# Kronuz/Xapiand

Measured on AMD Instinct MI355X. Metric: queries/sec + p50 latency, 10M-doc synthetic index, 3-term AND, top-10, higher is better.
Workload: dtype u32 postings + f64 BM25

## Files before the change

include/xgm.h:

```cpp
#ifndef XGM_H
#define XGM_H

#include <stddef.h>
#include <stdint.h>

#ifdef __cplusplus
extern "C" {
#endif
#if defined(__GNUC__)
#pragma GCC visibility push(default)
#endif

#define XGM_MAX_TERMS 16
#define XGM_MAX_K 1024

#define XGM_OK 0
#define XGM_UNSUPPORTED 1
#define XGM_E_INVALID (-1)
#define XGM_E_IO (-2)
#define XGM_E_NO_DEVICE (-3)
#define XGM_E_DEVICE (-4)
#define XGM_E_REVISION (-5)
#define XGM_E_NOMEM (-6)

// ... 349 lines not shown
int xgm_last_batch_bitmap_skipped(xgm_index*, uint64_t* words);

uint64_t xgm_query_postings_bytes(const xgm_index*, const xgm_query*);

int64_t xgm_debug_decode_term_device(xgm_index*, uint32_t term_id, uint32_t* did, uint32_t* wdf, uint64_t cap);

int64_t xgm_debug_read_doclen(xgm_index*, uint32_t* out, uint64_t cap);

int64_t xgm_debug_read_positions(xgm_index*, uint32_t term_id, uint32_t* out, uint64_t cap);

int64_t xgm_debug_read_container(xgm_index*, uint32_t term_id, uint32_t stripe, unsigned char* out, uint64_t cap, uint32_t* layout);

int xgm_debug_read_wdf_summary(xgm_index*, uint32_t term_id, uint32_t stripe, uint64_t* out);

int xgm_debug_read_term_wdf0(xgm_index*, uint32_t term_id, uint32_t* out);

int64_t xgm_debug_read_flat(xgm_index*, uint32_t term_id, uint32_t* did, unsigned char* wdf, uint32_t* pos, uint64_t cap, uint32_t* has_pos);

double xgm_debug_plan_us(const xgm_index*, const xgm_query_desc* descs, const xgm_global_stats* gs, uint32_t nq, uint32_t reps);

int xgm_debug_batch_launches(const xgm_index*, const xgm_query* qs, uint32_t nq, char* out, uint32_t cap);

int xgm_debug_host_ns(uint64_t* out8);

int xgm_debug_replay_info(uint64_t* out2);
typedef struct {
    uint64_t known_matching_docs;
    double max_weight, frozen_weight;
    uint32_t n_hits, max_weight_subqs, frozen, parallel;
} xgm_replay_figures;
int xgm_debug_replay_list(int device, const xgm_hit* list, uint64_t n, uint32_t k, uint64_t check_at_least, uint32_t mode, uint64_t seg_min,
                          xgm_hit* hits, xgm_replay_figures* out);
int xgm_debug_batch_replay_info(uint64_t* out3);
int xgm_debug_batching_info(const xgm_index*, uint64_t* out3);
double xgm_debug_concurrent_searches(xgm_index*, const xgm_query_desc* descs, const xgm_global_stats* gs, uint32_t n,
                                     uint32_t n_threads, uint32_t per_thread, uint32_t k, double* lat_us);

int xgm_debug_phase_cycles(unsigned long long* out8);
int xgm_debug_merge_cycles(unsigned long long* out8);
int xgm_debug_orw_phase_cycles(unsigned long long* out8);
int64_t xgm_debug_plan_batch(const xgm_index*, const xgm_query* qs, uint32_t nq, char* kernel, uint32_t* units, uint64_t cap);
int xgm_debug_or_bounds(const xgm_index*, const xgm_query* q, double* seed, double* ub, double* ub1);
int xgm_debug_set_plan_facts(xgm_index* idx, uint64_t dense_min_df, uint32_t flags, uint64_t flat_postings);
int64_t xgm_debug_plan_dump(const xgm_index*, const xgm_query* qs, uint32_t nq, uint32_t mode, uint32_t force_general, uint64_t* out, uint32_t cap);
int64_t xgm_debug_last_units(xgm_index*, unsigned long long* out, uint64_t cap);
int64_t xgm_debug_last_units2(xgm_index*, unsigned long long* out, unsigned long long* out_pos, uint64_t cap);

const char* xgm_last_error(void);
const char* xgm_version(void);

#if defined(__GNUC__)
#pragma GCC visibility pop
#endif
#ifdef __cplusplus
}
#endif
#endif
```

xapiand_amd/_lib.py:

```python
import ctypes as C
import os

XGM_MAX_TERMS = 16
XGM_MAX_TREE = 40
XGM_OP_TREE = 8
XGM_MAX_K = 1024
XGM_OK, XGM_UNSUPPORTED = 0, 1
XGM_E_INVALID, XGM_E_IO, XGM_E_NO_DEVICE, XGM_E_DEVICE, XGM_E_REVISION, XGM_E_NOMEM = -1, -2, -3, -4, -5, -6
XGM_OP_AND, XGM_OP_OR, XGM_OP_PHRASE = 1, 2, 3
XGM_OP_AND_NOT, XGM_OP_AND_MAYBE, XGM_OP_FILTER, XGM_OP_NEAR = 4, 5, 6, 7
XGM_REPLAY_BATCH_COUNT = 2
XGM_REPLAY_BATCH_FROZEN = 1
XGM_KNOWN_LOWER_BOUND = 1 << 63
XGM_ALL_NOT_A_MATCH = 0x80000000
XGM_MATCHES_LOWER_BOUND = 1 << 63
XGM_DEVICE_NONE = -1
UINT64_MAX = (1 << 64) - 1

_HERE = os.path.dirname(os.path.abspath(__file__))
LIB_PATH = os.environ.get("XGM_LIB_PATH") or os.path.join(_HERE, "csrc", "libxgm.so")


class RawPostings(C.Structure):
    _fields_ = [("n_terms", C.c_uint32), ("lastdocid", C.c_uint32), ("doccount", C.c_uint32),
# ... 125 lines not shown
    ("xgm_debug_filter_batch_info", C.c_int, [_P(C.c_uint64)]),
    ("xgm_filter_combine", C.c_int, [C.c_void_p, C.c_uint32, C.c_void_p, C.c_void_p, _P(C.c_void_p), _P(C.c_uint64)]),
    ("xgm_filter_all", C.c_int, [C.c_void_p, _P(C.c_void_p), _P(C.c_uint64)]),
    ("xgm_index_attach_live", C.c_int, [C.c_void_p, _P(C.c_uint32), C.c_uint32]),
    ("xgm_index_attach_live_file", C.c_int, [C.c_void_p, C.c_char_p]),
    ("xgm_glass_export_live", C.c_int, [C.c_char_p, C.c_char_p]),
    ("xgm_debug_live_info", C.c_int, [C.c_void_p, _P(C.c_uint64)]),
    ("xgm_search_filtered", C.c_int, [C.c_void_p, _P(Query), C.c_void_p, _P(SortSpec), _P(Hit), _P(C.c_uint32), _P(ResultHdr), C.c_int32, _P(C.c_uint32), C.c_uint32]),
    ("xgm_search_filtered_batch", C.c_int, [C.c_void_p, _P(Query), C.c_uint32, C.c_void_p, _P(SortSpec), C.c_uint32, _P(Hit), _P(C.c_uint32), _P(ResultHdr),
                                   C.c_int32, _P(C.c_uint32), C.c_uint32]),
    ("xgm_search_range", C.c_int, [C.c_void_p, C.c_void_p, _P(SortSpec), C.c_uint32, _P(Hit), _P(C.c_uint32), _P(ResultHdr), C.c_int32, _P(C.c_uint32), C.c_uint32]),
    ("xgm_filter_count_pairs", C.c_int, [C.c_void_p, C.c_void_p, C.c_uint32, C.c_uint32, _P(PairCount), C.c_uint64, _P(C.c_uint64)]),
    ("xgm_debug_pairs_info", C.c_int, [_P(C.c_uint64)]),
    ("xgm_segment_refresh_from_glass", C.c_int, [C.c_char_p, C.c_char_p, C.c_uint32, C.c_uint32, C.c_char_p]),
    ("xgm_glass_export_raw", C.c_int, [C.c_char_p, C.c_char_p]),
    ("xgm_glass_info", C.c_int, [C.c_char_p, _P(C.c_uint64), _P(C.c_uint32), _P(C.c_uint32), _P(C.c_uint64)]),
    ("xgm_segment_decode_term", C.c_int64, [C.c_char_p, C.c_char_p, C.c_size_t, _P(C.c_uint32), _P(C.c_uint32), C.c_uint64]),
    ("xgm_index_open", C.c_int, [C.c_char_p, C.c_int, C.c_uint64, _P(C.c_void_p)]),
    ("xgm_index_build_synthetic", C.c_int, [_P(SynthParams), C.c_int, _P(C.c_void_p)]),
    ("xgm_index_close", None, [C.c_void_p]),
    ("xgm_index_save", C.c_int, [C.c_void_p, C.c_char_p]),
    ("xgm_index_get_info", C.c_int, [C.c_void_p, _P(IndexInfo)]),
    ("xgm_index_set_stream", C.c_int, [C.c_void_p, C.c_void_p]),
    ("xgm_lookup_term", C.c_int, [C.c_void_p, C.c_char_p, C.c_size_t, _P(C.c_uint32), _P(C.c_uint32), _P(C.c_uint32), _P(C.c_uint32)]),
    ("xgm_index_termfreqs", C.c_int, [C.c_void_p, _P(C.c_uint32), C.c_uint32]),
    ("xgm_plan_query", C.c_int, [C.c_void_p, _P(QueryDesc), _P(GlobalStats), _P(Query)]),
    ("xgm_mset_bounds", None, [_P(Query), _P(ResultHdr), _P(C.c_uint32), _P(C.c_uint32), _P(C.c_uint32)]),
    ("xgm_search", C.c_int, [C.c_void_p, _P(Query), _P(Hit), _P(ResultHdr)]),
    ("xgm_search_all", C.c_int, [C.c_void_p, _P(Query), _P(Hit), C.c_uint64, _P(C.c_uint64), _P(ResultHdr)]),
    ("xgm_search_replay", C.c_int, [C.c_void_p, _P(Query), C.c_uint32, _P(Hit), _P(ResultHdr), _P(C.c_uint64)]),
    ("xgm_debug_replay_info", C.c_int, [_P(C.c_uint64)]),
    ("xgm_debug_replay_list", C.c_int, [C.c_int, _P(Hit), C.c_uint64, C.c_uint32, C.c_uint64, C.c_uint32, C.c_uint64, _P(Hit), _P(ReplayFigures)]),
    ("xgm_debug_batch_replay_info", C.c_int, [_P(C.c_uint64)]),
    ("xgm_search_batch", C.c_int, [C.c_void_p, _P(Query), C.c_uint32, C.c_uint32, _P(Hit), _P(ResultHdr)]),
    ("xgm_search_batch_known", C.c_int, [C.c_void_p, _P(Query), C.c_uint32, C.c_uint32, _P(Hit), _P(ResultHdr), _P(C.c_uint64)]),
    ("xgm_search_batch_begin", C.c_int, [C.c_void_p, _P(Query), C.c_uint32, C.c_uint32, _P(C.c_void_p)]),
    ("xgm_get_mset_batch_begin", C.c_int, [C.c_void_p, _P(QueryDesc), _P(GlobalStats), C.c_uint32, C.c_uint32, _P(C.c_void_p)]),
    ("xgm_batch_end", C.c_int, [C.c_void_p, _P(_P(Hit)), _P(_P(ResultHdr))]),
    ("xgm_batch_known", C.c_int, [C.c_void_p, _P(_P(C.c_uint64))]),
    ("xgm_batch_poll", C.c_int, [C.c_void_p]),
    ("xgm_batch_release", None, [C.c_void_p]),
    ("xgm_search_batch_device", C.c_int, [C.c_void_p, _P(Query), C.c_uint32, C.c_uint32, C.c_void_p, C.c_void_p]),
    ("xgm_get_mset_batch", C.c_int, [C.c_void_p, _P(QueryDesc), _P(GlobalStats), C.c_uint32, C.c_uint32, _P(Hit), _P(ResultHdr)]),
    ("xgm_get_mset_batch_device", C.c_int, [C.c_void_p, _P(QueryDesc), _P(GlobalStats), C.c_uint32, C.c_uint32, C.c_void_p, C.c_void_p]),
    ("xgm_search_sharded", C.c_int, [_P(C.c_void_p), C.c_uint32, _P(QueryDesc), C.c_uint32, C.c_uint32, _P(Hit), _P(ResultHdr)]),
    ("xgm_debug_sharded_info", C.c_int, [C.c_void_p, _P(C.c_uint64)]),
    ("xgm_merge_shards_device", C.c_int, [C.c_void_p, C.c_void_p, C.c_void_p, C.c_uint32, C.c_uint32, C.c_uint32, _P(C.c_uint32), C.c_void_p, C.c_void_p]),
    ("xgm_merge_shards_packed_device", C.c_int, [C.c_void_p, C.c_void_p, C.c_uint32, C.c_uint32, C.c_uint32, _P(C.c_uint32), C.c_void_p, C.c_void_p]),
    ("xgm_shard_record_bytes", C.c_size_t, [C.c_uint32, C.c_uint32]),
    ("xgm_index_set_profiling", C.c_int, [C.c_void_p, C.c_int]),
    ("xgm_index_set_near_colocated", C.c_int, [C.c_void_p, C.c_int]),
    ("xgm_last_kernel_ms", C.c_double, [C.c_void_p]),
    ("xgm_last_kernel_name", C.c_char_p, [C.c_void_p]),
    ("xgm_last_batch_traffic", C.c_int, [C.c_void_p, _P(C.c_uint64), C.c_uint32]),
    ("xgm_last_batch_bitmap_skipped", C.c_int, [C.c_void_p, _P(C.c_uint64)]),
    ("xgm_query_postings_bytes", C.c_uint64, [C.c_void_p, _P(Query)]),
    ("xgm_debug_decode_term_device", C.c_int64, [C.c_void_p, C.c_uint32, _P(C.c_uint32), _P(C.c_uint32), C.c_uint64]),
    ("xgm_debug_read_doclen", C.c_int64, [C.c_void_p, _P(C.c_uint32), C.c_uint64]),
    ("xgm_debug_read_positions", C.c_int64, [C.c_void_p, C.c_uint32, _P(C.c_uint32), C.c_uint64]),
    ("xgm_debug_read_container", C.c_int64, [C.c_void_p, C.c_uint32, C.c_uint32, _P(C.c_ubyte), C.c_uint64, _P(C.c_uint32)]),
    ("xgm_debug_read_wdf_summary", C.c_int, [C.c_void_p, C.c_uint32, C.c_uint32, _P(C.c_uint64)]),
    ("xgm_debug_read_term_wdf0", C.c_int, [C.c_void_p, C.c_uint32, _P(C.c_uint32)]),
    ("xgm_debug_read_flat", C.c_int64, [C.c_void_p, C.c_uint32, _P(C.c_uint32), _P(C.c_ubyte), _P(C.c_uint32), C.c_uint64, _P(C.c_uint32)]),
    ("xgm_debug_plan_us", C.c_double, [C.c_void_p, _P(QueryDesc), _P(GlobalStats), C.c_uint32, C.c_uint32]),
    ("xgm_debug_batch_launches", C.c_int, [C.c_void_p, _P(Query), C.c_uint32, C.c_char_p, C.c_uint32]),
    ("xgm_index_set_batching", C.c_int, [C.c_void_p, C.c_uint32]),
# ... 65 lines not shown
```

xapiand_amd/csrc/xgm_api.cc:

```cpp
#include <hip/hip_runtime.h>

#include <algorithm>
#include <atomic>
#include <chrono>
#include <condition_variable>
#include <deque>
#include <thread>
#include <cstdarg>
#include <cstdlib>
#include <cmath>
#include <cstring>
#include <string>

#include "xgm_batch_plan.h"
#include "xgm_filter_hold.h"
#include "xgm_internal.h"
#include "xgm_launch.h"

int xgm_read_segment_file(const char* path, XgmSegmentBlob* blob);


static thread_local char g_err[512] = "";

int xgm_set_error(int code, const char* fmt, ...) {
// ... 27 lines not shown
}


struct XgmScratch {
    hipStream_t stream = nullptr;
    xgm_dev_query* d_queries = nullptr;
    xgm_cand* d_cand = nullptr; size_t cap_cand = 0;
    xgm_group_hdr* d_ghdr = nullptr; size_t cap_ghdr = 0;
    uint32_t* d_kq = nullptr; double* d_maxposs = nullptr;
    uint32_t* d_mkq = nullptr; size_t cap_mkq = 0;
    uint32_t* d_hist = nullptr; size_t cap_hist = 0;
    xgm_work* d_work = nullptr;
    uint32_t* d_goff = nullptr;
    void* d_in = nullptr; size_t cap_in = 0;
    xgm_hit* d_hits = nullptr; size_t cap_hits = 0;
    xgm_result_hdr* d_hdrs = nullptr; size_t cap_hdrs = 0;
    unsigned char* d_sorted = nullptr; size_t cap_sorted = 0;
    void* h_sorted = nullptr; size_t cap_hsorted = 0;
    xgm_hit* d_part_hits = nullptr; size_t cap_part_hits = 0;
    xgm_result_hdr* d_part_hdrs = nullptr; size_t cap_part_hdrs = 0;
    xgm_hit* d_arena = nullptr; size_t cap_arena = 0;
    unsigned char* d_count = nullptr; size_t cap_count = 0;
    unsigned char* d_all = nullptr; size_t cap_all = 0;
    bool inorder = false;
    bool arrive_dirty = false;
    uint32_t* d_arrive = nullptr; size_t cap_arrive = 0;
    unsigned char* d_fbatch = nullptr;
    void* h_up = nullptr; size_t cap_up = 0;
    void* h_down = nullptr; size_t cap_down = 0;
    void* h_work = nullptr; size_t cap_hwork = 0;
    hipEvent_t ev0 = nullptr, ev1 = nullptr;
    hipEvent_t last_stop = nullptr;
    hipEvent_t ev_done = nullptr;
    bool pending = false;
};

template <class T>
static int grow(T** p, size_t* cap, size_t need) {
    if (need <= *cap) return XGM_OK;
    if (*p) HIP_TRY(hipFree(*p));
    *p = nullptr;
    size_t n = std::max(need + need / 2, *cap * 2);
    HIP_TRY(hipMalloc((void**)p, n * sizeof(T)));
    *cap = n;
    return XGM_OK;
}

static int grow_pinned(void** p, size_t* cap, size_t need) {
    if (need <= *cap) return XGM_OK;
    if (*p) HIP_TRY(hipHostFree(*p));
    *p = nullptr;
    size_t n = std::max(need + need / 2, *cap * 2);
    HIP_TRY(hipHostMalloc(p, n, hipHostMallocDefault));
    *cap = n;
    return XGM_OK;
}

#define XGM_MAX_SCRATCH 8u

static int scratch_acquire(xgm_index* idx, XgmScratch** out) {
    *out = nullptr;
    XgmScratch* wait_for = nullptr;
    {
        std::lock_guard<std::mutex> lk(idx->scratch_mu);
        std::vector<XgmScratch*>& pool = idx->scratch_pool;
        for (size_t i = pool.size(); i-- > 0;) {
            XgmScratch* c = pool[i];
            if (!c->pending || hipEventQuery(c->ev_done) == hipSuccess) {
                c->pending = false;
                c->inorder = false;
                pool.erase(pool.begin() + (ptrdiff_t)i);
                *out = c;
                break;
            }
        }
        const uint32_t depth = idx->stream ? 3u : XGM_MAX_SCRATCH;
        if (!*out && !pool.empty() && idx->scratch_total >= depth) {
            wait_for = pool.front();
            pool.erase(pool.begin());
        }
        if (!*out && !wait_for) ++idx->scratch_total;
    }
    if (*out) return XGM_OK;
    if (wait_for) {
        hipEventSynchronize(wait_for->ev_done);
        wait_for->pending = false;
        wait_for->inorder = false;
        *out = wait_for;
        return XGM_OK;
    }
    XgmScratch* s = new XgmScratch();
    hipError_t e = hipStreamCreateWithFlags(&s->stream, hipStreamNonBlocking);
    if (e != hipSuccess) {
        delete s;
        std::lock_guard<std::mutex> lk(idx->scratch_mu);
        --idx->scratch_total;
        return xgm_launch_error("hipStreamCreate", (int)e, hipGetErrorString(e));
    }
    hipEventCreate(&s->ev0);
    hipEventCreate(&s->ev1);
    hipEventCreateWithFlags(&s->ev_done, hipEventDisableTiming);
    *out = s;
    return XGM_OK;
}

static void scratch_release(xgm_index* idx, XgmScratch* s) {
    std::lock_guard<std::mutex> lk(idx->scratch_mu);
    idx->scratch_pool.push_back(s);
}

static void scratch_destroy(XgmScratch* s) {
    if (!s) return;
    hipFree(s->d_cand); hipFree(s->d_ghdr); hipFree(s->d_in); hipFree(s->d_mkq); hipFree(s->d_hist);
    hipFree(s->d_arena); hipFree(s->d_count);
    hipFree(s->d_hits); hipFree(s->d_hdrs); hipFree(s->d_part_hits); hipFree(s->d_part_hdrs); hipFree(s->d_arrive); hipFree(s->d_sorted); hipFree(s->d_all);
    hipFree(s->d_fbatch);
    if (s->h_sorted) hipHostFree(s->h_sorted);
    if (s->h_up) hipHostFree(s->h_up);
    if (s->h_down) hipHostFree(s->h_down);
    if (s->h_work) hipHostFree(s->h_work);
    if (s->ev0) hipEventDestroy(s->ev0);
    if (s->ev1) hipEventDestroy(s->ev1);
    if (s->ev_done) hipEventDestroy(s->ev_done);
    if (s->stream) hipStreamDestroy(s->stream);
    delete s;
}

static int next_event_pair(xgm_index* idx, hipEvent_t* start, hipEvent_t* stop) {
    *start = *stop = nullptr;
    if (!idx->profiling) return XGM_OK;
    std::lock_guard<std::mutex> lk(idx->scratch_mu);
    if (idx->prof_used == idx->prof_events.size()) {
        hipEvent_t a = nullptr, b = nullptr;
        if (hipEventCreate(&a) != hipSuccess || hipEventCreate(&b) != hipSuccess) {
            if (a) hipEventDestroy(a);
            return xgm_launch_error("profiling events", 0, "hipEventCreate");
        }
        idx->prof_events.push_back({a, b});
    }
    *start = (hipEvent_t)idx->prof_events[idx->prof_used].first;
    *stop = (hipEvent_t)idx->prof_events[idx->prof_used].second;
    ++idx->prof_used;
    return XGM_OK;
}


void xgm_shard_ctx_destroy(XgmShardCtx* c);
void xgm_batcher_destroy(xgm_index* idx);

static void fill_view(xgm_index* idx) {
    xgm_seg_dev& v = idx->view;
    v.doclen = (const uint32_t*)idx->d_sections[XGM_S_DOCLEN];
    v.term_blk = (const uint64_t*)idx->d_sections[XGM_S_TERM_BLK];
    v.term_word = (const uint64_t*)idx->d_sections[XGM_S_TERM_WORD];
    v.term_pos = (const uint64_t*)idx->d_sections[XGM_S_TERM_POS];
    v.blk_first = (const uint32_t*)idx->d_sections[XGM_S_BLK_FIRST];
    v.blk_meta = (const uint32_t*)idx->d_sections[XGM_S_BLK_META];
    v.blk_word = (const uint32_t*)idx->d_sections[XGM_S_BLK_WORD];
    v.blk_pos = (const uint32_t*)idx->d_sections[XGM_S_BLK_POS];
    v.words = (const uint32_t*)idx->d_sections[XGM_S_WORDS];
    v.positions = (const unsigned char*)idx->d_sections[XGM_S_POSITIONS];
    v.term_flags = (const uint32_t*)idx->d_sections[XGM_S_TERM_FLAGS];
    v.stripe_bits = idx->hdr.stripe_bits;
    v.lastdocid = idx->hdr.lastdocid;
    v.dense_id = nullptr; v.dense_dir = nullptr; v.dense_data = nullptr; v.n_dense = 0; v.dense_pos = 0; v.dense_plane = 0;
    v.dense_p2 = nullptr; v.bit_screen = 0; v.exact_wdf = 0; v.dense_wdf0 = nullptr; v.staged_bitmaps = 0; v.reserved_ = 0;
    v.doclen_narrow = nullptr; v.doclen_narrow_bits = 0; v.doclen_base = 0;
    v.flat_off = nullptr; v.flat_did = nullptr; v.flat_wdf = nullptr; v.flat_pos = nullptr;
    v.n_stripes = (idx->hdr.lastdocid >> idx->hdr.stripe_bits) + 1u;
}

static void adopt_host_dictionary(xgm_index* idx, const XgmSegmentBlob& blob) {
    const xgm_seg_header* h = blob.header();
    const uint32_t T = h->n_terms;
    idx->term_df.assign(blob.section<uint32_t>(XGM_S_TERM_DF), blob.section<uint32_t>(XGM_S_TERM_DF) + T);
    idx->term_cf.assign(blob.section<uint32_t>(XGM_S_TERM_CF), blob.section<uint32_t>(XGM_S_TERM_CF) + T);
// ... 99 lines not shown
}

extern "C" int xgm_index_get_info(const xgm_index* idx, xgm_index_info* out) {
    if (!idx || !out) return xgm_set_error(XGM_E_INVALID, "null argument");
    const xgm_seg_header& h = idx->hdr;
    out->n_terms = h.n_terms; out->lastdocid = h.lastdocid; out->doccount = h.doccount; out->has_positions = h.has_positions;
    out->total_length = h.total_length; out->revision = h.revision; out->n_postings = h.n_postings;
    out->n_positions = h.n_positions; out->n_blocks = h.n_blocks;
    out->device_bytes = idx->device_bytes;
    out->payload_bytes = h.n_words * 4;
    out->stripe_bits = h.stripe_bits; out->block_size = h.block_size;
    out->doclen_lower_bound = h.doclen_lower_bound; out->wdf_upper_bound = h.wdf_upper_bound;
    return XGM_OK;
}

extern "C" int xgm_index_set_stream(xgm_index* idx, void* hip_stream) {
    if (!idx) return xgm_set_error(XGM_E_INVALID, "null argument");
    idx->stream = hip_stream;
    idx->own_stream = false;
    return XGM_OK;
}

extern "C" int xgm_index_set_near_colocated(xgm_index* idx, int may_exist) {
    if (!idx) return xgm_set_error(XGM_E_INVALID, "null argument");
    idx->near_colocated.store(may_exist != 0);
    return XGM_OK;
}

extern "C" int xgm_index_set_profiling(xgm_index* idx, int on) {
    if (!idx) return xgm_set_error(XGM_E_INVALID, "null argument");
    std::lock_guard<std::mutex> lk(idx->scratch_mu);
    idx->profiling = (on & 1) != 0;
    idx->tally = (on & 2) != 0;
    idx->prof_used = 0;
    return XGM_OK;
}

extern "C" double xgm_last_kernel_ms(const xgm_index* cidx) {
    xgm_index* idx = const_cast<xgm_index*>(cidx);
    if (!idx) return -1.0;
    std::lock_guard<std::mutex> lk(idx->scratch_mu);
    if (idx->prof_used == 0) return -1.0;
    double sum = 0.0;
    size_t n = 0;
    for (size_t i = 0; i < idx->prof_used; ++i) {
        hipEvent_t a = (hipEvent_t)idx->prof_events[i].first, b = (hipEvent_t)idx->prof_events[i].second;
        float ms = 0.f;
        if (hipEventSynchronize(b) == hipSuccess && hipEventElapsedTime(&ms, a, b) == hipSuccess) { sum += ms; ++n; }
    }
    idx->prof_used = 0;
    return n ? sum / (double)n : -1.0;
}

extern "C" const char* xgm_last_kernel_name(const xgm_index* idx) { return idx ? idx->last_kernel : ""; }


static inline uint64_t term_hash(const char* p, size_t n) {
    uint64_t h = 0x9E3779B97F4A7C15ull ^ (n * 0xFF51AFD7ED558CCDull);
    while (n >= 8) { uint64_t v; memcpy(&v, p, 8); h = (h ^ v) * 0xD6E8FEB86659FD93ull; h ^= h >> 32; p += 8; n -= 8; }
    uint64_t v = 0;
    memcpy(&v, p, n);
    h = (h ^ v) * 0xD6E8FEB86659FD93ull;
    return h ^ (h >> 29);
}

static void build_term_hash(xgm_index* idx) {
    const uint32_t T = idx->hdr.n_terms;
// ... 135 lines not shown
        o_cur = 0; o_tab = 64;
        o_state = o_tab + (((size_t)bp.n_work * XGM_ALL_CHUNKS * 4 + 63) & ~(size_t)63);
        o_before = o_state + ((size_t)bp.n_work + nq) * bp.k_stride_c * sizeof(xgm_cand);
        o_ver = o_before + (size_t)bp.n_work * 8;
        if ((rc = grow(&s->d_count, &s->cap_count, o_ver + (size_t)bp.n_work * 4))) return rc;
        all_out.arena = s->d_arena; all_out.cursor = (unsigned long long*)(s->d_count + o_cur); all_out.cap = std::min<unsigned long long>(arena_entries, 0xFFFFFFFFull);
        all_out.chunk_tab = (uint32_t*)(s->d_count + o_tab);
        HIP_TRY(hipMemsetAsync(s->d_count, 0, 64, stream));
    }
    if ((rc = grow(&s->d_cand, &s->cap_cand, (size_t)bp.n_work * bp.k_stride_c))) return rc;
    if ((rc = grow(&s->d_ghdr, &s->cap_ghdr, (size_t)bp.n_work))) return rc;
    const uint32_t P = bp.parts, npq = nq * P;
    const size_t o_dq = 0, b_dq = (size_t)nq * sizeof(xgm_dev_query);
    const size_t o_mp = o_dq + b_dq, b_mp = (size_t)npq * 8;
    const size_t o_wk = o_mp + b_mp, b_wk = (size_t)bp.n_work * sizeof(xgm_work);
    const size_t o_kq = o_wk + b_wk, b_kq = (size_t)npq * 4;
    const size_t o_go = o_kq + b_kq, b_go = ((size_t)npq + 1) * 4;
    const size_t o_ro = o_go + b_go, b_ro = rows ? (size_t)nq * 4 : 0;
    const size_t o_fu = (o_ro + b_ro + 15) & ~(size_t)15, b_fu = sizeof(xgm_fuse);
    const size_t in_bytes = (o_fu + b_fu + 15) & ~(size_t)15;
    if ((rc = grow_pinned(&s->h_work, &s->cap_hwork, in_bytes))) return rc;
    if ((rc = grow(reinterpret_cast<unsigned char**>(&s->d_in), &s->cap_in, in_bytes))) return rc;
    unsigned char* hin = (unsigned char*)s->h_work;
    memcpy(hin + o_dq, h_dq, b_dq);
    for (uint32_t p = 0; p < P; ++p) { memcpy(hin + o_mp + (size_t)p * nq * 8, h_mp, (size_t)nq * 8); memcpy(hin + o_kq + (size_t)p * nq * 4, h_kq, (size_t)nq * 4); }
    memcpy(hin + o_wk, bp.work.data(), b_wk);
    memcpy(hin + o_go, bp.goff.data(), b_go);
    if (rows) memcpy(hin + o_ro, rows, b_ro);
    bool dense = mode == 0 && bp.andw && !bp.wide && bp.sided == 0 && bp.stripes_per_group <= xgm_dense_max_stripes();
    for (uint32_t i = 0; i < nq && dense; ++i) dense = xgm_dense_kind(idx, qs[i]) == (bp.phrase ? 2 : 1);
    static const bool dense_class_old_kernel = getenv("XGM_DENSE_CLASS_OLD_KERNEL") != nullptr;
    if (dense_class_old_kernel) dense = false;
    const bool fused = bp.fused;
    {
        unsigned char* din_ = (unsigned char*)s->d_in;
        xgm_fuse fu;
        memset(&fu, 0, sizeof fu);
        if (fused) {
            const size_t cap_before = s->cap_arrive;
            if ((rc = grow(&s->d_arrive, &s->cap_arrive, (size_t)std::max<uint32_t>(nq, 1024u)))) return rc;
            if (s->cap_arrive != cap_before || s->arrive_dirty) HIP_TRY(hipMemsetAsync(s->d_arrive, 0, s->cap_arrive * sizeof(uint32_t), stream));
            s->arrive_dirty = true;
            static const bool poison = getenv("XGM_DEBUG_POISON_SCRATCH") != nullptr;
            if (poison) {
                HIP_TRY(hipMemsetAsync(s->d_cand, 0, (size_t)bp.n_work * bp.k_stride_c * sizeof(xgm_cand), stream));
                HIP_TRY(hipMemsetAsync(s->d_ghdr, 0, (size_t)bp.n_work * sizeof(xgm_group_hdr), stream));
            }
            fu.arrive = s->d_arrive; fu.goff = (const uint32_t*)(din_ + o_go); fu.max_possible = (const double*)(din_ + o_mp);
            fu.row_of = rows ? (const uint32_t*)(din_ + o_ro) : nullptr;
            fu.hits = d_hits; fu.hdrs = d_hdrs; fu.k_stride_out = k_stride;
        }
        if (list) fu.goff = (const uint32_t*)(din_ + o_go);
        memcpy(hin + o_fu, &fu, sizeof fu);
    }
    const uint64_t t_cp = now_ns();
    g_host_ns[4] += t_cp - t_st;
    bool hist_zeroed = false;
    if (stream != s->stream && !s->inorder) {
        if (bp.orw || (bp.andw && bp.phrase)) {
            const size_t n_hist = list ? (size_t)bp.n_work : (size_t)nq * XGM_OR_HIST;
            if ((rc = grow(&s->d_hist, &s->cap_hist, n_hist))) return rc;
            HIP_TRY(hipMemsetAsync(s->d_hist, 0, n_hist * 4, s->stream));
            hist_zeroed = true;
        }
        HIP_TRY(hipMemcpyAsync(s->d_in, hin, in_bytes, hipMemcpyHostToDevice, s->stream));
        HIP_TRY(hipEventRecord(s->ev0, s->stream));
        HIP_TRY(hipStreamWaitEvent(stream, s->ev0, 0));
    } else {
        HIP_TRY(hipMemcpyAsync(s->d_in, hin, in_bytes, hipMemcpyHostToDevice, stream));
    }
    const uint64_t t_up = now_ns();
    g_host_ns[5] += t_up - t_cp;
    unsigned char* din = (unsigned char*)s->d_in;
    s->d_queries = (xgm_dev_query*)(din + o_dq);
    s->d_maxposs = (double*)(din + o_mp);
    s->d_work = (xgm_work*)(din + o_wk);
    s->d_kq = (uint32_t*)(din + o_kq);
    s->d_goff = (uint32_t*)(din + o_go);

    xgm_match_launch L;
    L.seg = idx->view;
    L.queries = s->d_queries;
    L.nq = nq; L.n_work = bp.n_work; L.work = s->d_work; L.stripes_per_group = bp.stripes_per_group; L.sub_bits = bp.sub_bits;
    static const bool debug_units = getenv("XGM_DEBUG_UNITS") != nullptr;
    if (debug_units && nq > 1) { g_last_work = bp.work; g_last_ghdr = s->d_ghdr; }
    L.tab_terms = bp.tab_terms; L.cap = bp.cap; L.k_stride = bp.k_stride_c;
    L.phrase = bp.phrase; L.wide = bp.wide; L.sided = bp.andw ? bp.sided : 0; L.orw2 = bp.orw2; L.orw_planes = bp.orw_planes; L.or_flat = bp.or_flat;
    L.tally = idx->tally;
    L.cand = s->d_cand; L.ghdr = s->d_ghdr;
    hipEvent_t pe0 = nullptr, pe1 = nullptr;
    if ((rc = next_event_pair(idx, &pe0, &pe1))) return rc;
    idx->last_kernel = xgm_plan_kernel_name(bp, mode, dense).name;
    idx->last_ghdr = s->d_ghdr; idx->last_n_work = bp.n_work;
    idx->last_tallied = idx->tally;
    if (idx->tally) {
        idx->last_staged_slots.clear();
        if (mode == 0 && bp.andw && !bp.phrase)
            for (uint32_t i = 0; i < bp.n_work; ++i)
                if (h_dq[bp.work[i].qi].flags & XGM_QF_DENSE) idx->last_staged_slots.push_back(bp.work[i].slot);
    }
    if (bp.orw || (bp.andw && bp.phrase)) {
        if (!hist_zeroed) {
            const size_t n_hist = list ? (size_t)bp.n_work : (size_t)nq * XGM_OR_HIST;
            if ((rc = grow(&s->d_hist, &s->cap_hist, n_hist))) return rc;
            HIP_TRY(hipMemsetAsync(s->d_hist, 0, n_hist * 4, stream));
        }
        L.hist = s->d_hist;
    }
    if (fused || list) L.fuse = (const xgm_fuse*)(din + o_fu);
    static const bool ext_launch = getenv("XGM_NO_EXT_LAUNCH") == nullptr;
    const bool ext = ext_launch && !dense && (bp.andw || (bp.orw && !bp.orw2));
    s->last_stop = nullptr;
    if (ext) {
        L.ev_start = pe0;
        L.ev_stop = pe1 ? pe1 : (fused ? s->ev1 : nullptr);
        if (fused) s->last_stop = L.ev_stop;
        pe0 = pe1 = nullptr;
    }
    if (pe0) HIP_TRY(hipEventRecord(pe0, stream));
    if ((rc = all ? xgm_launch_andw_all(L, all_out, stream) : list ? xgm_launch_andw_list(L, stream) : dense ? xgm_launch_dense(L, stream) : bp.andw ? xgm_launch_andw(L, stream)
              : bp.orw ? xgm_launch_orw(L, s->d_hist, stream)
              : bp.and_only ? xgm_launch_and(L, stream) : xgm_launch_match(L, stream)))
        return rc;
    if (pe1) HIP_TRY(hipEventRecord(pe1, stream));
    const uint64_t t_mk = now_ns();
    g_host_ns[6] += t_mk - t_up;
    const uint32_t* d_rows = rows ? (const uint32_t*)(din + o_ro) : nullptr;
    if (list) {
        if ((rc = xgm_launch_frozen_finish(s->d_queries, nq, s->d_goff, s->d_cand, s->d_ghdr, bp.k_stride_c, s->d_maxposs, d_rows, d_hits, d_hdrs, d_extra, k_stride, stream)))
            return rc;
    } else if (all) {
        if ((rc = xgm_launch_count_finish(s->d_queries, nq, s->d_work, bp.n_work, s->d_goff, s->d_cand, s->d_ghdr, bp.k_stride_c, all_out, (xgm_cand*)(s->d_count + o_state),
                                          (uint32_t*)(s->d_count + o_ver), (unsigned long long*)(s->d_count + o_before), s->d_maxposs, d_rows, d_hits, d_hdrs, d_extra, k_stride, stream)))
            return rc;
    } else if (fused) {
    } else if (P == 1u) {
        if ((rc = xgm_launch_merge(s->d_cand, s->d_ghdr, s->d_goff, bp.k_stride_c, s->d_kq, nq, bp.merge_cap, k_stride, d_hits,
                                   d_hdrs, s->d_maxposs, d_rows, stream)))
            return rc;
    } else {
        if ((rc = grow(&s->d_part_hits, &s->cap_part_hits, (size_t)npq * k_stride))) return rc;
        if ((rc = grow(&s->d_part_hdrs, &s->cap_part_hdrs, (size_t)npq))) return rc;
        if ((rc = xgm_launch_merge(s->d_cand, s->d_ghdr, s->d_goff, bp.k_stride_c, s->d_kq, npq, bp.merge_cap, k_stride, s->d_part_hits,
                                   s->d_part_hdrs, s->d_maxposs, nullptr, stream)))
            return rc;
        if ((rc = xgm_launch_merge_parts(s->d_part_hits, s->d_part_hdrs, P, nq, k_stride, s->d_kq, std::max(256u, xgm_next_pow2(P * k_stride)), d_hits, d_hdrs,
                                         d_rows, stream)))
            return rc;
    }
    g_host_ns[7] += now_ns() - t_mk;
// ... 82 lines not shown
    if (nq == 1 && idx->batcher) return batcher_submit(idx, qs, k_stride, hits, hdrs, known);
    return search_batch_now(idx, qs, nq, k_stride, hits, hdrs, known);
}

struct xgm_inflight {
    xgm_index* idx = nullptr;
    XgmScratch* s = nullptr;
    uint32_t nq = 0, k_stride = 0;
    bool ended = false;
    int rc_end = XGM_OK;
    bool has_extra = false;
    std::vector<xgm_query> plans;
    std::vector<uint32_t> host_replay;
};

static int batch_begin(xgm_index* idx, const xgm_query* qs, uint32_t nq, uint32_t k_stride, xgm_inflight** out, hipStream_t on = nullptr, bool inorder = false) {
    *out = nullptr;
    int rc = use_device(idx->device);
    if (rc) return rc;
    XgmScratch* s;
    if ((rc = scratch_acquire(idx, &s))) return rc;
    hipStream_t stream = on ? on : pick_stream(idx, s);
    s->inorder = inorder;
    bool has_extra = false;
    for (uint32_t i = 0; i < nq && !has_extra; ++i) has_extra = qs[i].replay != 0u;
    std::vector<uint32_t> host_replay;
    do {
        const size_t n_hit = (size_t)nq * k_stride;
        if ((rc = grow(&s->d_hits, &s->cap_hits, n_hit + (size_t)nq * 2 + (has_extra ? (nq + 1u) / 2u : 0u)))) break;
        xgm_result_hdr* d_hdrs = reinterpret_cast<xgm_result_hdr*>(s->d_hits + n_hit);
        unsigned long long* d_extra = has_extra ? reinterpret_cast<unsigned long long*>(s->d_hits + n_hit + (size_t)nq * 2) : nullptr;
        const size_t down = n_hit * sizeof(xgm_hit) + (size_t)nq * sizeof(xgm_result_hdr) + (has_extra ? (size_t)nq * 8 : 0);
        if ((rc = grow_pinned(&s->h_down, &s->cap_down, down))) break;
        if (has_extra) {
            const hipError_t ez = hipMemsetAsync(d_extra, 0, (size_t)nq * 8, stream);
            if (ez != hipSuccess) { rc = xgm_launch_error("hipMemsetAsync", (int)ez, hipGetErrorString(ez)); break; }
        }
        if ((rc = run_batch(idx, s, stream, qs, nq, k_stride, s->d_hits, d_hdrs, d_extra, has_extra ? &host_replay : nullptr))) break;
        static const bool copy_in_order = getenv("XGM_COPY_ON_BATCH_STREAM") != nullptr;
        hipError_t e = hipSuccess;
        if (stream != s->stream && !copy_in_order && !s->inorder) {
            hipEvent_t after = s->last_stop;
            if (!after) { after = s->ev1; e = hipEventRecord(after, stream); }
            if (e == hipSuccess) e = hipStreamWaitEvent(s->stream, after, 0);
            if (e == hipSuccess) e = hipMemcpyAsync(s->h_down, s->d_hits, down, hipMemcpyDeviceToHost, s->stream);
            if (e == hipSuccess) e = hipEventRecord(s->ev_done, s->stream);
        } else {
            e = hipMemcpyAsync(s->h_down, s->d_hits, down, hipMemcpyDeviceToHost, stream);
            if (e == hipSuccess) e = hipEventRecord(s->ev_done, stream);
        }
        if (e != hipSuccess) { rc = xgm_launch_error("result copy", (int)e, hipGetErrorString(e)); break; }
    } while (0);
    if (rc) {
        hipStreamSynchronize(stream);
        hipStreamSynchronize(s->stream);
        scratch_release(idx, s);
        return rc;
    }
    xgm_inflight* f = new xgm_inflight();
    f->idx = idx; f->s = s; f->nq = nq; f->k_stride = k_stride;
    if (has_extra) { f->has_extra = true; f->plans.assign(qs, qs + nq); f->host_replay.swap(host_replay); }
    *out = f;
    return XGM_OK;
}

extern "C" int xgm_search_batch_begin(xgm_index* idx, const xgm_query* qs, uint32_t nq, uint32_t k_stride, xgm_inflight** out) {
    if (!idx || !qs || !out || nq == 0) return xgm_set_error(XGM_E_INVALID, "null argument");
    if (idx->device == XGM_DEVICE_NONE) return xgm_set_error(XGM_E_NO_DEVICE, "index opened without a device");
    return batch_begin(idx, qs, nq, k_stride, out);
}

extern "C" int xgm_get_mset_batch_begin(xgm_index* idx, const xgm_query_desc* descs, const xgm_global_stats* gs, uint32_t nq, uint32_t k_stride,
                                        xgm_inflight** out) {
    if (!idx || !descs || !out || nq == 0) return xgm_set_error(XGM_E_INVALID, "null argument");
    if (idx->device == XGM_DEVICE_NONE) return xgm_set_error(XGM_E_NO_DEVICE, "index opened without a device");
    static thread_local std::vector<xgm_query> plans;
    plans.resize(nq);
    const uint64_t t0 = now_ns();
    for (uint32_t i = 0; i < nq; ++i) {
        int rc = xgm_plan_query(idx, &descs[i], gs ? &gs[i] : nullptr, &plans[i]);
        if (rc) return rc;
    }
    g_host_ns[0] += now_ns() - t0;
    return batch_begin(idx, plans.data(), nq, k_stride, out);
}

static int batch_host_replays(xgm_inflight* f) {
    xgm_hit* h_hits = (xgm_hit*)f->s->h_down;
    xgm_result_hdr* h_hdrs = (xgm_result_hdr*)(h_hits + (size_t)f->nq * f->k_stride);
    unsigned long long* h_extra = (unsigned long long*)(h_hdrs + f->nq);
    for (uint32_t i = 0; i < f->nq; ++i) if (h_extra[i] & XGM_EXTRA_FALLBACK) { f->host_replay.push_back(i); ++g_batch_replays[1]; }
    if (f->host_replay.empty()) return XGM_OK;
    std::vector<xgm_hit> page(XGM_MAX_K);
    for (uint32_t i : f->host_replay) {
        const xgm_query& q = f->plans[i];
        const uint32_t k = q.first + q.maxitems;
        const bool device_declined = (h_extra[i] & XGM_EXTRA_FALLBACK) != 0ull;
        const bool positional = (q.op == XGM_OP_PHRASE || q.op == XGM_OP_NEAR) && q.phrase_active;
        const bool frozen = (q.replay & XGM_REPLAY_BATCH_FROZEN) && positional;
        h_extra[i] = 0;
        if (!frozen && !(q.replay & XGM_REPLAY_BATCH_COUNT)) continue;
        if (!device_declined && h_hdrs[i].n_hits < k && !(h_hdrs[i].matches_exact & XGM_MATCHES_LOWER_BOUND)) { h_extra[i] = h_hdrs[i].n_hits; continue; }
        xgm_result_hdr hdr;
        uint64_t known = 0;
        const int rc = xgm_search_replay(f->idx, &q, frozen ? XGM_REPLAY_FROZEN_WEIGHT : XGM_REPLAY_COUNT, page.data(), &hdr, &known);
        if (rc) return rc;
        ++g_batch_replays[2];
        h_extra[i] = known;
        if (!frozen && !device_declined) { h_hdrs[i].matches_exact = hdr.matches_exact; continue; }
        hdr.max_possible = q.max_possible;
        memcpy(h_hits + (size_t)i * f->k_stride, page.data(), (size_t)hdr.n_hits * sizeof(xgm_hit));
        h_hdrs[i] = hdr;
    }
    return XGM_OK;
}

extern "C" int xgm_batch_end(xgm_inflight* f, const xgm_hit** hits, const xgm_result_hdr** hdrs) {
    if (!f) return xgm_set_error(XGM_E_INVALID, "null argument");
    if (!f->ended) {
        f->ended = true;
        hipError_t e = hipEventSynchronize(f->s->ev_done);
        if (e != hipSuccess) f->rc_end = xgm_launch_error("batch completion", (int)e, hipGetErrorString(e));
        else if (f->has_extra) f->rc_end = batch_host_replays(f);
    }
    if (hits) *hits = (const xgm_hit*)f->s->h_down;
    if (hdrs) *hdrs = (const xgm_result_hdr*)((const xgm_hit*)f->s->h_down + (size_t)f->nq * f->k_stride);
    return f->rc_end;
}

extern "C" int xgm_batch_known(xgm_inflight* f, const uint64_t** known) {
    if (!f || !known) return xgm_set_error(XGM_E_INVALID, "null argument");
    *known = nullptr;
    if (!f->ended) return xgm_set_error(XGM_E_INVALID, "xgm_batch_known before xgm_batch_end");
    if (f->has_extra) *known = (const uint64_t*)((const xgm_result_hdr*)((const xgm_hit*)f->s->h_down + (size_t)f->nq * f->k_stride) + f->nq);
    return f->rc_end;
}

extern "C" int xgm_batch_poll(xgm_inflight* f) {
    if (!f) return xgm_set_error(XGM_E_INVALID, "null argument");
    if (f->ended) return 1;
    return hipEventQuery(f->s->ev_done) == hipSuccess ? 1 : 0;
}

extern "C" void xgm_batch_release(xgm_inflight* f) {
    if (!f) return;
    if (!f->ended) hipEventSynchronize(f->s->ev_done);
    scratch_release(f->idx, f->s);
    delete f;
}

static int search_batch_now(xgm_index* idx, const xgm_query* qs, uint32_t nq, uint32_t k_stride, xgm_hit* hits, xgm_result_hdr* hdrs, uint64_t* known) {
    xgm_inflight* f = nullptr;
    int rc = batch_begin(idx, qs, nq, k_stride, &f);
    if (rc) return rc;
    const xgm_hit* h_hits = nullptr;
    const xgm_result_hdr* h_hdrs = nullptr;
    rc = xgm_batch_end(f, &h_hits, &h_hdrs);
    if (rc == XGM_OK) {
        memcpy(hdrs, h_hdrs, (size_t)nq * sizeof(xgm_result_hdr));
        for (uint32_t i = 0; i < nq; ++i)
            memcpy(hits + (size_t)i * k_stride, h_hits + (size_t)i * k_stride, (size_t)h_hdrs[i].n_hits * sizeof(xgm_hit));
        const uint64_t* kn = nullptr;
        if (known && xgm_batch_known(f, &kn) == XGM_OK && kn) memcpy(known, kn, (size_t)nq * 8);
    }
    xgm_batch_release(f);
    return rc;
}


static int attach_ordinals(xgm_index* idx, uint32_t slot, const uint32_t* ord, size_t n_ord, uint32_t n_distinct);

extern "C" int xgm_index_attach_column(xgm_index* idx, const char* column_path) {
    if (!idx || !column_path) return xgm_set_error(XGM_E_INVALID, "null argument");
    if (idx->device == XGM_DEVICE_NONE) return xgm_set_error(XGM_E_NO_DEVICE, "index opened without a device");
    FILE* f = fopen(column_path, "rb");
    if (!f) return xgm_set_error(XGM_E_IO, "cannot open %s: %s", column_path, strerror(errno));
    char magic[8];
    uint32_t h32[4];
    std::vector<uint32_t> ord;
// ... 1956 lines not shown
```

xapiand_amd/csrc/xgm_internal.h:

```cpp
#ifndef XGM_INTERNAL_H
#define XGM_INTERNAL_H

#include <atomic>
#include <cstdarg>
#include <cstdint>
#include <cstdio>
#include <map>
#include <mutex>
#include <string>
#include <utility>
#include <vector>

#include "../../include/xgm.h"
#include "xgm_segment.h"

int xgm_set_error(int code, const char* fmt, ...) __attribute__((format(printf, 2, 3)));

struct XgmSegmentBlob {
    std::vector<uint8_t> bytes;
    const uint8_t* map = nullptr;
    size_t map_size = 0;
    XgmSegmentBlob() = default;
    XgmSegmentBlob(const XgmSegmentBlob&) = delete;
    XgmSegmentBlob& operator=(const XgmSegmentBlob&) = delete;
// ... 60 lines not shown
    std::vector<char> str_bytes;
    std::vector<uint32_t> term_hash;
    std::once_flag term_hash_once;
    void* d_blob = nullptr;
    void* d_sections[XGM_S_COUNT] = {};
    bool sections_owned = false;
    xgm_seg_dev view{};
    uint64_t device_bytes = 0;
    void* d_dense_id = nullptr;
    void* d_dense_dir = nullptr;
    void* d_dense_data = nullptr;
    void* d_dense_p2 = nullptr;
    void* d_dense_wdf0 = nullptr;
    void* d_doclen_narrow = nullptr;
    void* d_flat_off = nullptr;
    void* d_flat_did = nullptr;
    void* d_flat_wdf = nullptr;
    void* d_flat_pos = nullptr;
    uint64_t flat_bytes = 0;
    uint64_t dense_bytes = 0;
    XgmPlanFacts facts;
    void* stream = nullptr;
    bool own_stream = false;
    bool profiling = false;
    std::atomic<bool> near_colocated{false};
    bool tally = false;
    const char* last_kernel = "";
    void* last_ghdr = nullptr;
    uint32_t last_n_work = 0;
    bool last_tallied = false;
    std::vector<uint32_t> last_staged_slots;
    std::vector<std::pair<void*, void*>> prof_events;
    size_t prof_used = 0;
    std::mutex scratch_mu;
    std::vector<XgmScratch*> scratch_pool;
    uint32_t scratch_total = 0;
    XgmBatcher* batcher = nullptr;
    XgmShardCtx* shard_ctx = nullptr;
    std::vector<XgmShardCtx*> retired_shard_ctx;
    std::map<uint32_t, std::pair<void*, uint32_t>> columns;
    std::vector<uint32_t> term_order;
    std::once_flag term_order_once;
    std::vector<void*> retired_columns;
    std::mutex columns_mu;
    struct ListColumn { void* head = nullptr; void* ext = nullptr; uint32_t n_distinct = 0; };
    std::map<uint32_t, ListColumn> list_columns;
    std::mutex live_mu;
    void* d_live = nullptr;
    uint32_t live_state = 0;
    uint32_t live_source = 0;
    uint32_t live_launches = 0;
    uint64_t live_marked = 0;
};

int xgm_lookup_term_id(const xgm_index* idx, const char* term, size_t len, uint32_t* id);

int xgm_build_dense(xgm_index* idx);

#endif
```

Measured before the change: 931,800.

## Write fused AND results directly into mapped pinned host memory, skipping download copy

For fused AND-weight batches launched off the scratch stream, the kernel now writes hits and headers straight into a device-mapped pinned host buffer. This removes the separate device-to-host copy and its cross-stream event wait, and completion is tracked by the kernel's stop event. Instead of making the compute stream wait on the upload event, the host briefly spins on the upload before launching. The change adds bookkeeping so profiling events that serve as completion markers are not reused early, and it risks slower kernel writes over PCIe/fabric to host memory.

New measurement: 1.002 million (median of 6 runs). +7.5%, better.

```diff
diff --git a/include/xgm.h b/include/xgm.h
--- a/include/xgm.h
+++ b/include/xgm.h
@@ -405,6 +405,7 @@
 int xgm_debug_replay_list(int device, const xgm_hit* list, uint64_t n, uint32_t k, uint64_t check_at_least, uint32_t mode, uint64_t seg_min,
                           xgm_hit* hits, xgm_replay_figures* out);
 int xgm_debug_batch_replay_info(uint64_t* out3);
+int xgm_debug_inflight_info(uint64_t* out2);
 int xgm_debug_batching_info(const xgm_index*, uint64_t* out3);
 double xgm_debug_concurrent_searches(xgm_index*, const xgm_query_desc* descs, const xgm_global_stats* gs, uint32_t n,
                                      uint32_t n_threads, uint32_t per_thread, uint32_t k, double* lat_us);
diff --git a/xapiand_amd/_lib.py b/xapiand_amd/_lib.py
--- a/xapiand_amd/_lib.py
+++ b/xapiand_amd/_lib.py
@@ -181,6 +181,7 @@
     ("xgm_debug_replay_info", C.c_int, [_P(C.c_uint64)]),
     ("xgm_debug_replay_list", C.c_int, [C.c_int, _P(Hit), C.c_uint64, C.c_uint32, C.c_uint64, C.c_uint32, C.c_uint64, _P(Hit), _P(ReplayFigures)]),
     ("xgm_debug_batch_replay_info", C.c_int, [_P(C.c_uint64)]),
+    ("xgm_debug_inflight_info", C.c_int, [_P(C.c_uint64)]),
     ("xgm_search_batch", C.c_int, [C.c_void_p, _P(Query), C.c_uint32, C.c_uint32, _P(Hit), _P(ResultHdr)]),
     ("xgm_search_batch_known", C.c_int, [C.c_void_p, _P(Query), C.c_uint32, C.c_uint32, _P(Hit), _P(ResultHdr), _P(C.c_uint64)]),
     ("xgm_search_batch_begin", C.c_int, [C.c_void_p, _P(Query), C.c_uint32, C.c_uint32, _P(C.c_void_p)]),
diff --git a/xapiand_amd/csrc/xgm_api.cc b/xapiand_amd/csrc/xgm_api.cc
--- a/xapiand_amd/csrc/xgm_api.cc
+++ b/xapiand_amd/csrc/xgm_api.cc
@@ -83,8 +83,17 @@
     hipEvent_t ev0 = nullptr, ev1 = nullptr;
     hipEvent_t last_stop = nullptr;
     hipEvent_t ev_done = nullptr;
+    hipEvent_t done = nullptr;
+    bool done_in_pool = false;
+    bool offer_host_rows = false;
+    bool host_rows = false;
+    void* h_down_dev = nullptr;
+    void* h_down_mapped = nullptr;
     bool pending = false;
 };
+
+static std::atomic<uint64_t> g_inflight_info[2];
+extern "C" int xgm_debug_inflight_info(uint64_t* out2) { if (!out2) return -1; for (int i = 0; i < 2; ++i) out2[i] = g_inflight_info[i].load(); return 0; }
 
 template <class T>
 static int grow(T** p, size_t* cap, size_t need) {
@@ -117,7 +126,7 @@
         std::vector<XgmScratch*>& pool = idx->scratch_pool;
         for (size_t i = pool.size(); i-- > 0;) {
             XgmScratch* c = pool[i];
-            if (!c->pending || hipEventQuery(c->ev_done) == hipSuccess) {
+            if (!c->pending || hipEventQuery(c->done) == hipSuccess) {
                 c->pending = false;
                 c->inorder = false;
                 pool.erase(pool.begin() + (ptrdiff_t)i);
@@ -134,7 +143,7 @@
     }
     if (*out) return XGM_OK;
     if (wait_for) {
-        hipEventSynchronize(wait_for->ev_done);
+        hipEventSynchronize(wait_for->done);
         wait_for->pending = false;
         wait_for->inorder = false;
         *out = wait_for;
@@ -151,6 +160,7 @@
     hipEventCreate(&s->ev0);
     hipEventCreate(&s->ev1);
     hipEventCreateWithFlags(&s->ev_done, hipEventDisableTiming);
+    s->done = s->ev_done;
     *out = s;
     return XGM_OK;
 }
@@ -177,14 +187,16 @@
     delete s;
 }
 
-static int next_event_pair(xgm_index* idx, hipEvent_t* start, hipEvent_t* stop) {
+static int next_event_pair(xgm_index* idx, hipEvent_t* start, hipEvent_t* stop, bool hold_for_rows = false) {
     *start = *stop = nullptr;
     if (!idx->profiling) return XGM_OK;
     std::lock_guard<std::mutex> lk(idx->scratch_mu);
+    if (hold_for_rows) ++idx->prof_rows_held;
     if (idx->prof_used == idx->prof_events.size()) {
         hipEvent_t a = nullptr, b = nullptr;
         if (hipEventCreate(&a) != hipSuccess || hipEventCreate(&b) != hipSuccess) {
             if (a) hipEventDestroy(a);
+            if (hold_for_rows) --idx->prof_rows_held;
             return xgm_launch_error("profiling events", 0, "hipEventCreate");
         }
         idx->prof_events.push_back({a, b});
@@ -193,6 +205,22 @@
     *stop = (hipEvent_t)idx->prof_events[idx->prof_used].second;
     ++idx->prof_used;
     return XGM_OK;
+}
+
+static void rewind_event_pairs(xgm_index* idx) {
+    if (idx->prof_rows_held)
+        for (size_t i = 0; i < idx->prof_used; ++i) hipEventSynchronize((hipEvent_t)idx->prof_events[i].second);
+    idx->prof_used = 0;
+}
+
+static void scratch_drop_rows_event(xgm_index* idx, XgmScratch* s) {
+    if (s->done_in_pool) {
+        std::lock_guard<std::mutex> lk(idx->scratch_mu);
+        --idx->prof_rows_held;
+        s->done_in_pool = false;
+    }
+    s->done = s->ev_done;
+    s->host_rows = s->offer_host_rows = false;
 }
 
 
@@ -358,7 +386,7 @@
     std::lock_guard<std::mutex> lk(idx->scratch_mu);
     idx->profiling = (on & 1) != 0;
     idx->tally = (on & 2) != 0;
-    idx->prof_used = 0;
+    rewind_event_pairs(idx);
     return XGM_OK;
 }
 
@@ -560,6 +588,10 @@
     static const bool dense_class_old_kernel = getenv("XGM_DENSE_CLASS_OLD_KERNEL") != nullptr;
     if (dense_class_old_kernel) dense = false;
     const bool fused = bp.fused;
+    static const bool ext_launch = getenv("XGM_NO_EXT_LAUNCH") == nullptr;
+    const bool ext = ext_launch && !dense && (bp.andw || (bp.orw && !bp.orw2));
+    const bool host_rows = s->offer_host_rows && fused && ext && bp.andw && mode == 0 && !rows;
+    s->host_rows = host_rows;
     {
         unsigned char* din_ = (unsigned char*)s->d_in;
         xgm_fuse fu;
@@ -577,6 +609,7 @@
             fu.arrive = s->d_arrive; fu.goff = (const uint32_t*)(din_ + o_go); fu.max_possible = (const double*)(din_ + o_mp);
             fu.row_of = rows ? (const uint32_t*)(din_ + o_ro) : nullptr;
             fu.hits = d_hits; fu.hdrs = d_hdrs; fu.k_stride_out = k_stride;
+            if (host_rows) { fu.hits = (xgm_hit*)s->h_down_dev; fu.hdrs = (xgm_result_hdr*)(fu.hits + (size_t)nq * k_stride); }
         }
         if (list) fu.goff = (const uint32_t*)(din_ + o_go);
         memcpy(hin + o_fu, &fu, sizeof fu);
@@ -584,6 +617,7 @@
     const uint64_t t_cp = now_ns();
     g_host_ns[4] += t_cp - t_st;
     bool hist_zeroed = false;
+    bool upload_awaited = false;
     if (stream != s->stream && !s->inorder) {
         if (bp.orw || (bp.andw && bp.phrase)) {
             const size_t n_hist = list ? (size_t)bp.n_work : (size_t)nq * XGM_OR_HIST;
@@ -593,7 +627,9 @@
         }
         HIP_TRY(hipMemcpyAsync(s->d_in, hin, in_bytes, hipMemcpyHostToDevice, s->stream));
         HIP_TRY(hipEventRecord(s->ev0, s->stream));
-        HIP_TRY(hipStreamWaitEvent(stream, s->ev0, 0));
+        static const bool wait_on_stream = getenv("XGM_UPLOAD_WAIT_ON_STREAM") != nullptr;
+        if (wait_on_stream || !host_rows) HIP_TRY(hipStreamWaitEvent(stream, s->ev0, 0));
+        else upload_awaited = true;
     } else {
         HIP_TRY(hipMemcpyAsync(s->d_in, hin, in_bytes, hipMemcpyHostToDevice, stream));
     }
@@ -617,7 +653,8 @@
     L.tally = idx->tally;
     L.cand = s->d_cand; L.ghdr = s->d_ghdr;
     hipEvent_t pe0 = nullptr, pe1 = nullptr;
-    if ((rc = next_event_pair(idx, &pe0, &pe1))) return rc;
+    if ((rc = next_event_pair(idx, &pe0, &pe1, host_rows))) return rc;
+    if (host_rows && pe1) s->done_in_pool = true;
     idx->last_kernel = xgm_plan_kernel_name(bp, mode, dense).name;
     idx->last_ghdr = s->d_ghdr; idx->last_n_work = bp.n_work;
     idx->last_tallied = idx->tally;
@@ -636,14 +673,21 @@
         L.hist = s->d_hist;
     }
     if (fused || list) L.fuse = (const xgm_fuse*)(din + o_fu);
-    static const bool ext_launch = getenv("XGM_NO_EXT_LAUNCH") == nullptr;
-    const bool ext = ext_launch && !dense && (bp.andw || (bp.orw && !bp.orw2));
     s->last_stop = nullptr;
     if (ext) {
         L.ev_start = pe0;
         L.ev_stop = pe1 ? pe1 : (fused ? s->ev1 : nullptr);
         if (fused) s->last_stop = L.ev_stop;
+        if (host_rows) s->done = L.ev_stop;
         pe0 = pe1 = nullptr;
+    }
+    if (upload_awaited) {
+        const uint64_t t_spin = now_ns();
+        hipError_t eu = hipEventQuery(s->ev0);
+        while (eu == hipErrorNotReady && now_ns() - t_spin < 200000ull) eu = hipEventQuery(s->ev0);
+        if (eu == hipErrorNotReady) eu = hipEventSynchronize(s->ev0);
+        if (eu != hipSuccess) return xgm_launch_error("upload", (int)eu, hipGetErrorString(eu));
+        ++g_inflight_info[1];
     }
     if (pe0) HIP_TRY(hipEventRecord(pe0, stream));
     if ((rc = all ? xgm_launch_andw_all(L, all_out, stream) : list ? xgm_launch_andw_list(L, stream) : dense ? xgm_launch_dense(L, stream) : bp.andw ? xgm_launch_andw(L, stream)
@@ -792,6 +836,18 @@
         unsigned long long* d_extra = has_extra ? reinterpret_cast<unsigned long long*>(s->d_hits + n_hit + (size_t)nq * 2) : nullptr;
         const size_t down = n_hit * sizeof(xgm_hit) + (size_t)nq * sizeof(xgm_result_hdr) + (has_extra ? (size_t)nq * 8 : 0);
         if ((rc = grow_pinned(&s->h_down, &s->cap_down, down))) break;
+        static const bool no_host_rows = getenv("XGM_NO_HOST_ROWS") != nullptr;
+        s->host_rows = false;
+        s->offer_host_rows = !no_host_rows && stream != s->stream && !s->inorder && !has_extra;
+        if (s->offer_host_rows && s->h_down_mapped != s->h_down) {
+#if defined(XGM_EMU)
+            s->h_down_dev = s->h_down;
+#else
+            const hipError_t em = hipHostGetDevicePointer(&s->h_down_dev, s->h_down, 0);
+            if (em != hipSuccess) { rc = xgm_launch_error("hipHostGetDevicePointer", (int)em, hipGetErrorString(em)); break; }
+#endif
+            s->h_down_mapped = s->h_down;
+        }
         if (has_extra) {
             const hipError_t ez = hipMemsetAsync(d_extra, 0, (size_t)nq * 8, stream);
             if (ez != hipSuccess) { rc = xgm_launch_error("hipMemsetAsync", (int)ez, hipGetErrorString(ez)); break; }
@@ -799,7 +855,10 @@
         if ((rc = run_batch(idx, s, stream, qs, nq, k_stride, s->d_hits, d_hdrs, d_extra, has_extra ? &host_replay : nullptr))) break;
         static const bool copy_in_order = getenv("XGM_COPY_ON_BATCH_STREAM") != nullptr;
         hipError_t e = hipSuccess;
-        if (stream != s->stream && !copy_in_order && !s->inorder) {
+        s->offer_host_rows = false;
+        if (s->host_rows) {
+            ++g_inflight_info[0];
+        } else if (stream != s->stream && !copy_in_order && !s->inorder) {
             hipEvent_t after = s->last_stop;
             if (!after) { after = s->ev1; e = hipEventRecord(after, stream); }
             if (e == hipSuccess) e = hipStreamWaitEvent(s->stream, after, 0);
@@ -814,6 +873,7 @@
     if (rc) {
         hipStreamSynchronize(stream);
         hipStreamSynchronize(s->stream);
+        scratch_drop_rows_event(idx, s);
         scratch_release(idx, s);
         return rc;
     }
@@ -879,7 +939,7 @@
     if (!f) return xgm_set_error(XGM_E_INVALID, "null argument");
     if (!f->ended) {
         f->ended = true;
-        hipError_t e = hipEventSynchronize(f->s->ev_done);
+        hipError_t e = hipEventSynchronize(f->s->done);
         if (e != hipSuccess) f->rc_end = xgm_launch_error("batch completion", (int)e, hipGetErrorString(e));
         else if (f->has_extra) f->rc_end = batch_host_replays(f);
     }
@@ -899,12 +959,13 @@
 extern "C" int xgm_batch_poll(xgm_inflight* f) {
     if (!f) return xgm_set_error(XGM_E_INVALID, "null argument");
     if (f->ended) return 1;
-    return hipEventQuery(f->s->ev_done) == hipSuccess ? 1 : 0;
+    return hipEventQuery(f->s->done) == hipSuccess ? 1 : 0;
 }
 
 extern "C" void xgm_batch_release(xgm_inflight* f) {
     if (!f) return;
-    if (!f->ended) hipEventSynchronize(f->s->ev_done);
+    if (!f->ended) hipEventSynchronize(f->s->done);
+    scratch_drop_rows_event(f->idx, f->s);
     scratch_release(f->idx, f->s);
     delete f;
 }
diff --git a/xapiand_amd/csrc/xgm_internal.h b/xapiand_amd/csrc/xgm_internal.h
--- a/xapiand_amd/csrc/xgm_internal.h
+++ b/xapiand_amd/csrc/xgm_internal.h
@@ -116,6 +116,7 @@
     std::vector<uint32_t> last_staged_slots;
     std::vector<std::pair<void*, void*>> prof_events;
     size_t prof_used = 0;
+    uint32_t prof_rows_held = 0;
     std::mutex scratch_mu;
     std::vector<XgmScratch*> scratch_pool;
     uint32_t scratch_total = 0;
```
